# ketanfatania/QMRI-PnP-Recon-POC

Measured on AMD Instinct MI355X. Metric: ADMM iters/sec (224x224x10 TSMI, spiral mask), higher is better.
Workload: dtype f32; 1 GPU; cut3 224x224x10 single slice per GPU, spiral mask S=771 T=200, PnP-ADMM + 10-channel UNetRes (DRUNet) denoiser; solver=lsqr, admm_iters=20, dc_dtype=f64, parallelism=slice-parallel x1 (no collective)

## Files before the change

### qmri_pnp_recon_poc_amd/csrc/api_core.cpp

```cpp
#include "qmri_internal.h"
#include "fft_codelets.h"

#include <algorithm>
#include <atomic>
#include <cmath>
#include <cstdarg>
#include <cstdlib>
#include <cstring>
#include <mutex>

static thread_local std::string g_create_err;

namespace {
struct KnobDef { const char* name; int dflt; };
const KnobDef g_knob_defs[K_COUNT] = {
    {"conv_scheme", 2}, {"conv_f32", 0}, {"conv_wt", 1}, {"conv_xcd", 1}, {"conv_persist", 1}, {"conv_splitk", 1},
    {"conv_midcfg", 3}, {"conv_deepcfg", 3}, {"conv_deepks", 4},
    {"conv_resident", 1}, {"res_head", 1}, {"res_tail", 1}, {"res_down", 1}, {"res_delay", 24}, {"res_rearm", 64},
    {"res_stamps", 0}, {"conv_stamps", 0}, {"conv_stamp_launch", -1}, {"lsqr_stamps", 0},
    {"conv_mt2", 1024}, {"conv_occ", 2},
    {"fuse_ew", 1}, {"lsqr_persist", 1}, {"lsqr_fold", 1}, {"dictw_lsp", 2}, {"verbose", 0},
    {"pack_gpu", 1}, {"nufft_seg", NU_SEG},
    {"fmap_fuse", 0}, {"fmap_start", 0},
};
std::atomic<int> g_knob_val[K_COUNT];
std::once_flag g_knob_once;

int knob_index(const char* name, size_t len) {
    for (int k = 0; k < K_COUNT; ++k)
        if (strlen(g_knob_defs[k].name) == len && strncmp(g_knob_defs[k].name, name, len) == 0) return k;
    return -1;
}
void knob_init() {
    for (int k = 0; k < K_COUNT; ++k) g_knob_val[k].store(g_knob_defs[k].dflt, std::memory_order_relaxed);
    const char* e = getenv("QMRI_DEBUG");
    while (e && *e) {
        const char* end = strchr(e, ',');
        const size_t len = end ? (size_t)(end - e) : strlen(e);
        const char* eq = (const char*)memchr(e, '=', len);
        const int k = eq ? knob_index(e, (size_t)(eq - e)) : -1;
        if (k >= 0) g_knob_val[k].store(atoi(eq + 1), std::memory_order_relaxed);
// ... 822 lines not shown
```

### qmri_pnp_recon_poc_amd/csrc/api_net.cpp

```cpp
#include "qmri_internal.h"

#include <algorithm>
#include <chrono>
#include <cmath>
#include <cstdio>
#include <cstring>

extern "C" size_t qmri_net_nparams(const qmri_net_desc* d) {
    if (!d) return 0;
    size_t n = 0;
    if (d->arch == QMRI_ARCH_UNETRES) {
        const int32_t* nc = d->nc;
        n += (size_t)nc[0] * d->in_nc * 9;
        for (int l = 0; l < 3; ++l) n += (size_t)2 * d->nb * nc[l] * nc[l] * 9 + (size_t)nc[l + 1] * nc[l] * 4;
        n += (size_t)2 * d->nb * nc[3] * nc[3] * 9;
        for (int l = 3; l > 0; --l) n += (size_t)nc[l] * nc[l - 1] * 4 + (size_t)2 * d->nb * nc[l - 1] * nc[l - 1] * 9;
        n += (size_t)d->out_nc * nc[0] * 9;
    } else if (d->arch == QMRI_ARCH_SEQ_CONV) {
        if (d->nb == 1) return (size_t)d->out_nc * d->in_nc * 9;
        n = (size_t)d->nc[0] * d->in_nc * 9 + (size_t)(d->nb - 2) * d->nc[0] * d->nc[0] * 9 + (size_t)d->out_nc * d->nc[0] * 9;
    }
    return n;
}

// ... 250 lines not shown
        for (int l = 0; l < 3; ++l) {
            for (int b = 0; b < 2 * nb; ++b) QMRI_TRY(add_layer_timed(ctx, CONV_3X3, nc[l], nc[l], w));
            QMRI_TRY(add_layer_timed(ctx, CONV_DOWN, nc[l], nc[l + 1], w));
        }
        for (int b = 0; b < 2 * nb; ++b) QMRI_TRY(add_layer_timed(ctx, CONV_3X3, nc[3], nc[3], w));
        for (int l = 3; l > 0; --l) {
            QMRI_TRY(add_layer_timed(ctx, CONV_UP, nc[l], nc[l - 1], w));
            for (int b = 0; b < 2 * nb; ++b) QMRI_TRY(add_layer_timed(ctx, CONV_3X3, nc[l - 1], nc[l - 1], w));
        }
        QMRI_TRY(add_layer_timed(ctx, CONV_3X3, nc[0], desc->out_nc, w));
        for (int l = 0; l < 4; ++l) {
            int cal = conv_cin_pad(CONV_3X3, nc[l]);
            if (l < 3) cal = std::max(cal, conv_cin_pad(CONV_DOWN, nc[l]));
            if (l > 0) cal = std::max(cal, conv_cin_pad(CONV_UP, nc[l]));
            QMRI_TRY(alloc_tensor(ctx, p.x[l], nc[l], cal, H >> l, W >> l, B));
            QMRI_TRY(alloc_tensor(ctx, p.a[l], nc[l], cal, H >> l, W >> l, B));
            QMRI_TRY(alloc_tensor(ctx, p.t[l], nc[l], cal, H >> l, W >> l, B));
        }
        if (nc[0] == 64 && H % 16 == 0 && W % 16 == 0 && (H / 16) * (W / 16) <= 1024) {
            p.res_tiles = (H / 16) * (W / 16);
            QMRI_TRY(dev_alloc(ctx, &p.d_res_xbuf, conv6r_xbuf_bytes(p.res_tiles)));
            QMRI_HIP(ctx, hipMemset(p.d_res_xbuf, 0, conv6r_xbuf_bytes(p.res_tiles)));
            p.res_epoch = 0; p.res_off = false;
            if (qmri_knob(K_RES_STAMPS)) { QMRI_HIP(ctx, hipMalloc(&p.d_res_stamps, 1024 * sizeof(unsigned long long))); QMRI_HIP(ctx, hipMemset(p.d_res_stamps, 0, 1024 * sizeof(unsigned long long))); }
        }
    } else {
        const int width = desc->nc[0];
        if (nb == 1) QMRI_TRY(add_layer_timed(ctx, CONV_3X3, desc->in_nc, desc->out_nc, w));
        else {
            QMRI_TRY(add_layer_timed(ctx, CONV_3X3, desc->in_nc, width, w));
            for (int l = 1; l < nb - 1; ++l) QMRI_TRY(add_layer_timed(ctx, CONV_3X3, width, width, w));
            QMRI_TRY(add_layer_timed(ctx, CONV_3X3, width, desc->out_nc, w));
        }
        QMRI_TRY(alloc_tensor(ctx, p.a[0], width, conv_cin_pad(CONV_3X3, width), H, W, B));
        QMRI_TRY(alloc_tensor(ctx, p.t[0], width, conv_cin_pad(CONV_3X3, width), H, W, B));
    }
    if (p.d_wflat) {
        const auto t0 = Clk::now();
        QMRI_TRY(net_pack_all_dev(ctx));
        QMRI_HIP(ctx, hipStreamSynchronize(ctx->stream));
        ms_pack += std::chrono::duration<double, std::milli>(Clk::now() - t0).count();
    }
    p.w_begin = nullptr;
    QMRI_TRY(alloc_tensor(ctx, p.in32, desc->in_nc, conv_cin_pad(CONV_3X3, desc->in_nc), H, W, B));
    QMRI_TRY(alloc_tensor(ctx, p.out32, desc->out_nc, desc->out_nc, H, W, B));
    p.blk_ok = conv6_enabled();
    for (const ConvLayer& L : p.layers) if (!L.wp6) p.blk_ok = false;
// ... 231 lines not shown
    auto pass = [&]() -> int {
        if (hipMemcpyAsync(d_io, in, nin * sizeof(double), hipMemcpyHostToDevice, ctx->stream) != hipSuccess) return QMRI_ERR_HIP;
        QMRI_TRY(ew_launch_pack(ctx, B, C, H, W, d_io, 1, p.in32, in_scale));
        QMRI_TRY(net_forward(ctx, B));
        QMRI_TRY(ew_launch_unpack(ctx, B, p.desc.out_nc, H, W, p.out32, p.in32, p.desc.residual_noise, d_io, 1, out_scale));
        if (hipMemcpyAsync(out, d_io, nout * sizeof(double), hipMemcpyDeviceToHost, ctx->stream) != hipSuccess) return QMRI_ERR_HIP;
        if (hipStreamSynchronize(ctx->stream) != hipSuccess) return QMRI_ERR_HIP;
        return net_range_tripped(ctx, again);
    };
    int st = QMRI_OK;
    for (int attempt = 0; attempt < 3; ++attempt) {
        again = false;
        st = pass();
        if (st != QMRI_OK || !again) break;
    }
    if (st == QMRI_OK && again) { qmri_set_error(ctx, "the network's guards asked for a fourth pass (resident-tile hand-off / f16 range): giving up"); st = QMRI_ERR_HIP; }
    if (st == QMRI_ERR_HIP && ctx->err.empty()) qmri_set_error(ctx, "HIP failure in qmri_denoise");
    return st;
}

extern "C" int qmri_debug_conv_stamps(qmri_ctx* ctx, unsigned long long* out, int nwg) {
    if (ctx && nwg == -6 && ctx->net.d_res_stamps) {
        QMRI_HIP(ctx, hipStreamSynchronize(ctx->stream));
        QMRI_HIP(ctx, hipMemcpy(out, ctx->net.d_res_stamps, (size_t)1024 * sizeof(unsigned long long), hipMemcpyDeviceToHost));
        return QMRI_OK;
    }
    if (!ctx || !ctx->net.d_stamps) return QMRI_ERR_STATE;
    QMRI_HIP(ctx, hipStreamSynchronize(ctx->stream));
    QMRI_HIP(ctx, hipMemcpy(out, ctx->net.d_stamps, (size_t)4096 * 11 * sizeof(unsigned long long), hipMemcpyDeviceToHost));
    return QMRI_OK;
}
```

### qmri_pnp_recon_poc_amd/csrc/conv6r_kernels.hip

```cpp
#include "conv6_device.h"

namespace {

constexpr int R_MAXL = 10;
constexpr int R_RELU = 1;
constexpr int R_ADD = 2;
constexpr int R_SKIP = 4;
constexpr int R_STORE = 8;
constexpr int R_STORE_WT = 16;
constexpr int R_KEEP = 32;
constexpr int R_DOWN = 128;
constexpr unsigned R_DOWN_STEPB = 2 * 2 * 2 * 64 * 16;
constexpr int R_LOCAL = 256;
constexpr int R_TAIL = 64;
constexpr int R_IH = 18, R_IW = 18, R_IHP = 24;
constexpr int R_NPX = R_IHP * (R_IW - 1) + R_IH;
constexpr int R_CHUNK = 2 * 2 * R_NPX;
constexpr int R_AST = ast6(2);
constexpr int R_SPIN_MAX = 1 << 16;
constexpr int R_SEGT = 86, R_CORT = 6;
constexpr int R_NTRI = 4 * R_SEGT + 4 * R_CORT;
constexpr size_t conv6r_lds() { return (size_t)(NABUF * R_AST + 4 * R_CHUNK) * 16; }

struct Conv6rArgs {
    const float* src; const float* skip;
    const float* radd[R_MAXL]; float* sdst[R_MAXL];
    float* dn_out; int dn_hp, dn_plane;
    float* out; int out_hp, out_plane, out_c;
    int in_planar, in_plane;
    int nch[R_MAXL], kind[R_MAXL];
    unsigned char* xbuf; size_t xbuf_half;
    const uint4* wp[R_MAXL];
    float dh[R_MAXL], dl[R_MAXL];
    int am_layer[R_MAXL];
    int nlayers, hp, plane, tiles_h, tiles_w, xcd;
    int drop;
    int delay;
    unsigned epoch;
    unsigned* range_flag; float* am_slots; int* am_count;
    unsigned long long* stamps;
};

template <int N> __device__ __forceinline__ void gwait_a(u32x4 (&a)[3]) { asm volatile("s_waitcnt vmcnt(%3)" : "+v"(a[0]), "+v"(a[1]), "+v"(a[2]) : "n"(N) : "memory"); }
template <int IMM> __device__ __forceinline__ void gload4r_sc1(f32x4& dst, unsigned off, const void* base) { asm volatile("global_load_dwordx4 %0, %1, %2 offset:%3 sc1" : "=v"(dst) : "v"(off), "s"(base), "n"(IMM) : "memory"); }
template <int IMM> __device__ __forceinline__ void gstore4r(unsigned off, f32x4 x, void* base) { asm volatile("global_store_dwordx4 %0, %1, %2 offset:%3\n\ts_nop 1" ::"v"(off), "v"(x), "s"(base), "n"(IMM) : "memory"); }
template <int IMM> __device__ __forceinline__ void gstore4r_sc1(unsigned off, f32x4 x, void* base) { asm volatile("global_store_dwordx4 %0, %1, %2 offset:%3 sc1\n\ts_nop 1" ::"v"(off), "v"(x), "s"(base), "n"(IMM) : "memory"); }

__device__ __forceinline__ void r_tri_decode(int t, int& seg, int& j) {
    if (t < 4 * R_SEGT) { seg = t / R_SEGT; j = t - seg * R_SEGT; } else { seg = 4 + (t - 4 * R_SEGT) / R_CORT; j = (t - 4 * R_SEGT) - (seg - 4) * R_CORT; }
}
__device__ __forceinline__ int r_seg_base(int seg) { return seg < 4 ? seg * R_SEGT : 4 * R_SEGT + (seg - 4) * R_CORT; }
__device__ __forceinline__ unsigned r_ent_lds(int k, int dw, int dh) {
    const int cb = k >> 1, sp = k & 1;
    return (unsigned)(((cb >> 1) * R_CHUNK + sp * 2 * R_NPX + (cb & 1) * R_NPX + dw * R_IHP + dh) * 16);
}

#define R_STAMP(role, k)                                                                                         \
    do {                                                                                                         \
        if constexpr (STAMP) {                                                                                   \
            if (A.stamps && (threadIdx.x & 255) == 0 && blockIdx.x % 50 == 0 && blockIdx.x / 50 < 4)             \
                A.stamps[(((blockIdx.x / 50) * 2 + (role)) * R_MAXL + l) * 8 + (k)] = wall_clock64();            \
        }                                                                                                        \
    } while (0)
template <bool STAMP>
__global__ __launch_bounds__(NT6) void k_conv6r(const Conv6rArgs A) {
    constexpr int SP = 2, AST = R_AST, IHP = R_IHP, NPX = R_NPX, NAQ = 3;
    static_assert(AST == NAQ * NLD6, "one weight step = three 16-byte entries per loader thread");
    extern __shared__ __align__(16) unsigned char smem[];
    uint4* Abuf = (uint4*)smem;
    uint4* Bt = Abuf + NABUF * AST;
    const int tid = threadIdx.x;
    const int bid = A.xcd ? xcd_remap(blockIdx.x, gridDim.x) : blockIdx.x;
    const int th = bid % A.tiles_h, tw = bid / A.tiles_h;
    const int oh0 = th * 16, ow0 = tw * 16;
    const int nl = A.nlayers;
    const unsigned plane32 = (unsigned)A.plane * 32u;
    const unsigned tile0 = (unsigned)((ow0 * A.hp + oh0) * 32);

    if (tid >= NT6 - NLD6) {
        const int lt = tid - (NT6 - NLD6);
        __builtin_amdgcn_s_setprio(2);
        constexpr unsigned ASTB = AST * 16;
        unsigned aoff[NAQ];
#pragma unroll
        for (int q = 0; q < NAQ; ++q) aoff[q] = (unsigned)((lt + NLD6 * q) * 16);
        int rq_l = 0, rq_s = 0, rq_n = 3 * A.nch[0];
// ... 72 lines not shown
                                   "+v"(v[2][2]), "+v"(v[2][3]), "+v"(v[2][4]), "+v"(v[2][5]), "+v"(v[2][6]), "+v"(v[2][7])::"memory");
#pragma unroll
                    for (int k = 0; k < NQ; ++k) {
                        uint4 s0, s1;
                        split_pair_h(v[k][0], v[k][1], s0.x, s1.x);
                        split_pair_h(v[k][2], v[k][3], s0.y, s1.y);
                        split_pair_h(v[k][4], v[k][5], s0.z, s1.z);
                        split_pair_h(v[k][6], v[k][7], s0.w, s1.w);
                        if (lo[k] != ~0u) {
                            *(uint4*)((unsigned char*)Bt + lo[k]) = s0;
                            *(uint4*)((unsigned char*)Bt + lo[k] + 2 * NPX * 16) = s1;
                        }
                    }
                }
            }
            gwait_a<0>(ra0); gwait_a<0>(pa1);
            R_STORE_A(0, ra0) R_STORE_A(1, pa1)
        }
        unsigned p_lds[2][3], p_x[2];
#pragma unroll
        for (int q = 0; q < 2; ++q) {
            const int t = lt + NLD6 * q;
            const bool valid = t < R_NTRI;
            int seg, j;
            r_tri_decode(valid ? t : 0, seg, j);
            const int npx = seg < 4 ? 16 : 1;
#pragma unroll
            for (int i = 0; i < 3; ++i) {
                const int E = 3 * j + i, Ec = (E < npx * 16) ? E : 0, pp = Ec >> 4, k = Ec & 15;
                const int w = (seg == 0) ? 0 : (seg == 1) ? 15 : (seg == 2 || seg == 3) ? pp : (seg < 6 ? 0 : 15);
                const int h = (seg == 0 || seg == 1) ? pp : (seg == 2) ? 0 : (seg == 3) ? 15 : ((seg & 1) ? 15 : 0);
                p_lds[q][i] = r_ent_lds(k, w + 1, h + 1);
            }
            p_x[q] = valid ? (unsigned)((tw * A.tiles_h + th) * (R_NTRI * 64) + t * 16) : ~0u;
        }
        lds_barrier6();
#define R_ITER(k_, rs_, rq_)               \
        {                                                                                                        \
            __builtin_amdgcn_s_setprio(2);                                                                       \
            R_REQ(rq_)                                                                                           \
            __builtin_amdgcn_s_setprio(0);                                                                       \
            gwait_a<2 * NAQ>(rs_);                                                                               \
            R_STORE_A(((k_) + 2) % NABUF, rs_)                                                                   \
            lds_barrier6();                                                                                      \
        }
#pragma unroll 1
        for (int l = 0; l < nl; ++l) {
#pragma unroll 1
            for (int g = 0; g < 3 * A.nch[l]; g += 3) {
                R_ITER(0, ra1, ra0)
                R_ITER(1, ra2, ra1)
                R_ITER(2, ra0, ra2)
            }
            R_STAMP(1, 0);
            if (A.kind[l] & R_TAIL) {
                lds_barrier6();
                const float* tl = (const float*)Bt;
                const unsigned opx = (unsigned)(((ow0 + (lt >> 4) + 1) * A.out_hp + (oh0 + (lt & 15)) + 1) * 4), opl = (unsigned)A.out_plane * 4u;
                for (int c = 0; c < A.out_c; ++c) {
                    const float x = tl[c * 256 + lt];
                    asm volatile("global_store_dword %0, %1, %2" ::"v"(opx + (unsigned)c * opl), "v"(x), "s"(A.out) : "memory");
                }
                break;
            }
            if (!(A.kind[l] & R_KEEP)) break;
            lds_barrier6();
            if (A.kind[l] & R_LOCAL) continue;
            R_STAMP(1, 1);
            const unsigned tag = (A.epoch + (unsigned)l + 1u) & 0xFFFFu, thi = tag << 16;
            unsigned char* xb = A.xbuf + (size_t)(l & 1) * A.xbuf_half;
            if (!(A.drop && th == 0 && tw == 0)) {
#pragma unroll
                for (int q = 0; q < 2; ++q) {
                    if (p_x[q] == ~0u) continue;
                    unsigned d[12];
#pragma unroll
                    for (int i = 0; i < 3; ++i) {
                        const uint4 e = *(const uint4*)((const unsigned char*)Bt + p_lds[q][i]);
                        d[4 * i] = e.x; d[4 * i + 1] = e.y; d[4 * i + 2] = e.z; d[4 * i + 3] = e.w;
                    }
#pragma unroll
                    for (int i = 0; i < 4; ++i) {
                        u32x4 g;
                        g[0] = d[3 * i];
                        g[1] = (d[3 * i + 1] & 0xFFFFu) | thi;
                        g[2] = (d[3 * i + 1] >> 16) | (d[3 * i + 2] << 16);
                        g[3] = (d[3 * i + 2] >> 16) | thi;
                        asm volatile("global_store_dwordx4 %0, %1, %2 sc1\n\ts_nop 1" ::"v"(p_x[q] + (unsigned)(i * (R_NTRI * 16))), "v"(g), "s"(xb) : "memory");
                    }
                }
            }
            R_STAMP(1, 2);
            R_STAMP(1, 5);
            lds_barrier6();
            R_STAMP(1, 6);
        }
        gwait_a<0>(ra0); gwait_a<0>(ra1); gwait_a<0>(ra2);
#undef R_ITER
#undef R_REQ
#undef R_STORE_A
        return;
    }
    const int wave = tid >> 6, lane = tid & 63, li = lane & 31, h2 = lane >> 5;
    const int pbw = 4 * wave;
    const int pxl = (pbw + (li >> 3)) * IHP + (li & 7);
    const unsigned gpx = (unsigned)(((ow0 + pbw + (li >> 3) + 1) * A.hp + (oh0 + (li & 7)) + 1) * 32 + 16 * h2);
    bool dead = false;
    lds_barrier6();
#pragma unroll 1
    for (int l = 0; l < nl; ++l) {
        R_STAMP(0, 0);
        f32x16 acc[2][2], accl[2][2];
#pragma unroll
        for (int m = 0; m < 2; ++m)
#pragma unroll
            for (int n = 0; n < 2; ++n)
#pragma unroll
// ... 144 lines not shown
                    go += plane32;                                                                               \
                }                                                                                                \
        }
#define R_ADD_OPERAND()                            \
        {                                                                                                        \
            asm volatile("s_waitcnt vmcnt(0)"                                                                    \
                         : "+v"(res[0][0][0]), "+v"(res[0][0][1]), "+v"(res[0][0][2]), "+v"(res[0][0][3]), "+v"(res[0][1][0]), "+v"(res[0][1][1]), \
                           "+v"(res[0][1][2]), "+v"(res[0][1][3]), "+v"(res[1][0][0]), "+v"(res[1][0][1]), "+v"(res[1][0][2]), "+v"(res[1][0][3]), \
                           "+v"(res[1][1][0]), "+v"(res[1][1][1]), "+v"(res[1][1][2]), "+v"(res[1][1][3])::"memory");     \
            _Pragma("unroll") for (int m = 0; m < 2; ++m)                                                        \
                _Pragma("unroll") for (int n = 0; n < 2; ++n)                                                    \
                    _Pragma("unroll") for (int r = 0; r < 16; r += 2) {                                          \
                        const f32x2 x = pair(m, n, r) + f32x2{res[m][n][r >> 2][r & 3], res[m][n][r >> 2][(r & 3) + 1]}; \
                        acc[m][n][r] = x[0]; acc[m][n][r + 1] = x[1];                                            \
                    }                                                                                            \
        }
        if (kind & R_ADD) { R_REQ_OPERAND(A.radd[l]) R_ADD_OPERAND() }
        if (kind & R_SKIP) { R_REQ_OPERAND(A.skip) R_ADD_OPERAND() }
#undef R_REQ_OPERAND
#undef R_ADD_OPERAND
        R_STAMP(0, 2);
        float gmax = 0.f;
        bool bad = false;
        auto finish = [&](auto relu_c, auto store_c, auto keep_c) __attribute__((always_inline)) {
            constexpr bool RELU = decltype(relu_c)::value, KEEP = decltype(keep_c)::value;
            constexpr int STORE = decltype(store_c)::value;
            float* sd = A.sdst[l];
            unsigned go = gpx_l;
#pragma unroll
            for (int m = 0; m < 2; ++m)
#pragma unroll
                for (int rg = 0; rg < 4; ++rg) {
#pragma unroll
                    for (int n = 0; n < 2; ++n) {
                        f32x4 x;
#pragma unroll
                        for (int j = 0; j < 4; ++j) { x[j] = acc[m][n][4 * rg + j]; if constexpr (RELU) x[j] = fmaxf(x[j], 0.f); }
                        const float gm = fmaxf(fmaxf(fabsf(x[0]), fabsf(x[1])), fmaxf(fabsf(x[2]), fabsf(x[3])));
                        bad |= !(gm <= F16_RANGE);
                        gmax = fmaxf(gmax, gm);
                        if constexpr (KEEP) {
                            uint2 s0, s1;
                            split_pair_h(x[0], x[1], s0.x, s1.x);
                            split_pair_h(x[2], x[3], s0.y, s1.y);
                            unsigned char* bd = (unsigned char*)Bt + (((2 * m + (rg >> 1)) * R_CHUNK + (rg & 1) * NPX + pxl_l + IHP + 1 + 8 * n) * 16 + 8 * h2_l);
                            *(uint2*)bd = s0;
                            *(uint2*)(bd + 2 * NPX * 16) = s1;
                        }
                        if constexpr (STORE != 0) {
                            if constexpr (STORE == 2) { if (n) gstore4r_sc1<256>(go, x, sd); else gstore4r_sc1<0>(go, x, sd); } else { if (n) gstore4r<256>(go, x, sd); else gstore4r<0>(go, x, sd); }
                        }
                    }
                    go += plane32;
                }
        };
        typedef std::true_type T1; typedef std::false_type T0;
        typedef std::integral_constant<int, 0> S0; typedef std::integral_constant<int, 1> S1; typedef std::integral_constant<int, 2> S2;
        if ((kind & R_RELU) && (kind & R_KEEP)) finish(T1{}, S0{}, T1{});
        else if ((kind & R_STORE) && (kind & R_KEEP)) finish(T0{}, S1{}, T1{});
        else if (kind & R_STORE_WT) finish(T0{}, S2{}, T0{});
        else finish(T0{}, S0{}, T1{});
        if (bad && A.range_flag) atomicOr(A.range_flag, 1u);
        act_report(ActMax{A.am_slots, A.am_count, A.am_layer[l]}, gmax, 4);
        R_STAMP(0, 3);
        if (!(kind & R_KEEP)) break;
        lds_barrier6();
        if (kind & R_LOCAL) continue;
        R_STAMP(0, 4);
        {
            int tid_l = tid;
            asm volatile("" : "+v"(tid_l));
            unsigned c_lds[2][3], c_x[2];
#pragma unroll
            for (int q = 0; q < 2; ++q) {
                const int t = tid_l + 256 * q;
                const bool valid = t < R_NTRI;
                int seg, j;
                r_tri_decode(valid ? t : 0, seg, j);
                const int npx = seg < 4 ? 16 : 1;
                const int dtw = (seg == 0 || seg == 4 || seg == 5) ? -1 : (seg == 1 || seg == 6 || seg == 7) ? 1 : 0;
                const int dth = (seg == 2 || seg == 4 || seg == 6) ? -1 : (seg == 3 || seg == 5 || seg == 7) ? 1 : 0;
                const int ns = (seg < 4) ? (seg ^ 1) : 11 - seg;
                const bool have = valid && tw + dtw >= 0 && tw + dtw < A.tiles_w && th + dth >= 0 && th + dth < A.tiles_h;
#pragma unroll
                for (int i = 0; i < 3; ++i) {
                    const int E = 3 * j + i, pp = E >> 4, k = E & 15;
                    const int dw = (dtw < 0) ? 0 : (dtw > 0) ? 17 : pp + 1, dh = (dth < 0) ? 0 : (dth > 0) ? 17 : pp + 1;
                    c_lds[q][i] = (have && E < npx * 16) ? r_ent_lds(k, dw, dh) : ~0u;
                }
                c_x[q] = have ? (unsigned)(((tw + dtw) * A.tiles_h + th + dth) * (R_NTRI * 64) + (r_seg_base(ns) + j) * 16) : ~0u;
            }
            const unsigned tag = (A.epoch + (unsigned)l + 1u) & 0xFFFFu, thi = tag << 16;
            const unsigned char* xb = A.xbuf + (size_t)(l & 1) * A.xbuf_half;
            for (int i = 0; i < A.delay; ++i) __builtin_amdgcn_s_sleep(1);
            {
                bool pend[2] = {c_x[0] != ~0u && !dead, c_x[1] != ~0u && !dead};
                bool ok = false;
                for (int spin = 0; spin < R_SPIN_MAX; ++spin) {
                    u32x4 g[2][4];
#pragma unroll
                    for (int q = 0; q < 2; ++q)
                        if (pend[q]) {
#pragma unroll
                            for (int i = 0; i < 4; ++i) asm volatile("global_load_dwordx4 %0, %1, %2 sc1" : "=v"(g[q][i]) : "v"(c_x[q] + (unsigned)(i * (R_NTRI * 16))), "s"(xb) : "memory");
                        }
                    asm volatile("s_waitcnt vmcnt(0)" : "+v"(g[0][0]), "+v"(g[0][1]), "+v"(g[0][2]), "+v"(g[0][3]), "+v"(g[1][0]), "+v"(g[1][1]), "+v"(g[1][2]), "+v"(g[1][3])::"memory");
#pragma unroll
                    for (int q = 0; q < 2; ++q)
                        if (pend[q]) {
                            unsigned bad = 0;
#pragma unroll
                            for (int i = 0; i < 4; ++i) bad |= (g[q][i][1] ^ thi) | (g[q][i][3] ^ thi);
                            if ((bad >> 16) == 0) {
                                unsigned d[12];
#pragma unroll
                                for (int i = 0; i < 4; ++i) {
                                    d[3 * i] = g[q][i][0];
                                    d[3 * i + 1] = (g[q][i][1] & 0xFFFFu) | (g[q][i][2] << 16);
                                    d[3 * i + 2] = (g[q][i][2] >> 16) | (g[q][i][3] << 16);
                                }
#pragma unroll
                                for (int i = 0; i < 3; ++i)
                                    if (c_lds[q][i] != ~0u) *(uint4*)((unsigned char*)Bt + c_lds[q][i]) = make_uint4(d[4 * i], d[4 * i + 1], d[4 * i + 2], d[4 * i + 3]);
                                pend[q] = false;
                            }
                        }
                    if (!__any(pend[0] || pend[1])) { ok = true; break; }
                    __builtin_amdgcn_s_sleep(1);
                }
                if (!ok && !dead) { dead = true; if (lane == 0 && A.range_flag) atomicOr(A.range_flag, 4u); }
            }
        }
        R_STAMP(0, 5);
        lds_barrier6();
        R_STAMP(0, 6);
    }
}

}

int conv6r_try(qmri_ctx* ctx, const Conv6rRun& run, int B, bool* done) {
    *done = false;
    NetPlan& net = ctx->net;
    hipStreamCaptureStatus cap = hipStreamCaptureStatusNone;
    const bool capturing = hipStreamIsCapturing(ctx->stream, &cap) == hipSuccess && cap != hipStreamCaptureStatusNone;
    const int nres = run.nres, nl = nres + (run.head ? 1 : 0) + (run.tail ? 1 : 0) + (run.down ? 1 : 0);
    if (!qmri_knob(K_CONV_RESIDENT) || capturing || net.res_off || !net.d_res_xbuf || B != 1 || nres < 2 || nl > R_MAXL || (nres & 1) || net.d_stamps) return QMRI_OK;
    if (!run.res || !run.src || !run.cur || (run.head && (!run.head_in || run.skip)) || (run.tail && !run.tail_out) || (run.down && (!run.down_out || run.tail || run.skip))) return QMRI_OK;
    auto is3 = [](const ConvLayer& L) { return (L.kind == CONV_3X3 || L.kind == CONV_3X3N) && L.sp6 == 2 && L.wp6 && L.n_ct6 == 1; };
    for (int l = 0; l < nres; ++l) {
        const ConvLayer& L = run.res[l];
        if (!is3(L) || L.Cin != 64 || L.Cout != 64 || L.nchunk6 != 4) return QMRI_OK;
    }
    const PTensor &src = *run.src, &cur = *run.cur;
    const PTensor* ts[3] = {&src, &cur, run.skip};
    for (const PTensor* t : ts) {
        if (!t) continue;
// ... 35 lines not shown
    int l = 0;
    auto put = [&](const ConvLayer& L, int kind, const float* radd, float* sdst) {
        A.wp[l] = reinterpret_cast<const uint4*>(L.wp6);
        A.dh[l] = L.w6_descale; A.dl[l] = L.w6_descale * (1.f / LO_SCALE);
        A.am_layer[l] = conv6_act_slot(ctx, true, L).layer;
        A.nch[l] = L.nchunk6; A.kind[l] = kind; A.radd[l] = radd; A.sdst[l] = sdst;
        ++l;
    };
    if (run.head) put(*run.head, R_STORE | R_KEEP, nullptr, src.fbase());
    for (int r = 0; r < nres; ++r) {
        const bool last = r == nres - 1;
        if (!(r & 1)) put(run.res[r], R_RELU | R_KEEP, nullptr, nullptr);
        else if (!last) put(run.res[r], R_ADD | R_STORE | R_KEEP, (r == 1) ? src.fbase() : cur.fbase(), cur.fbase());
        else if (run.tail) put(run.res[r], R_ADD | (run.skip ? R_SKIP : 0) | R_KEEP, (r == 1) ? src.fbase() : cur.fbase(), nullptr);
        else if (run.down) put(run.res[r], R_ADD | R_KEEP | R_LOCAL, (r == 1) ? src.fbase() : cur.fbase(), nullptr);
        else put(run.res[r], R_ADD | (run.skip ? R_SKIP : 0) | R_STORE_WT, (r == 1) ? src.fbase() : cur.fbase(), cur.fbase());
    }
    if (run.tail) put(*run.tail, R_TAIL, nullptr, nullptr);
    if (run.down) { put(*run.down, R_DOWN, nullptr, nullptr); A.nch[l - 1] = 6; }
    for (int k = l; k < R_MAXL; ++k) { A.wp[k] = A.wp[l - 1]; A.nch[k] = A.nch[l - 1]; A.am_layer[k] = -1; }
    int pub[2] = {0, 0};
    for (int k = 0; k < l; ++k) if ((A.kind[k] & R_KEEP) && !(A.kind[k] & R_LOCAL)) pub[k & 1] += 1;
    if (!pub[0] || !pub[1]) return QMRI_OK;
    A.nlayers = nl; A.hp = src.hp; A.plane = (int)src.plane(); A.tiles_h = tiles_h; A.tiles_w = tiles_w;
    A.xbuf = net.d_res_xbuf; A.xbuf_half = (size_t)tiles * R_NTRI * 64;
    A.xcd = qmri_knob(K_CONV_XCD);
    const int delay = std::max(0, std::min(4096, qmri_knob(K_RES_DELAY)));
    A.epoch = net.res_epoch; A.drop = net.res_drop; A.delay = delay;
    A.range_flag = net.d_range_flag; A.am_slots = net.d_act_slots; A.am_count = net.d_act_count;
    if (!ctx->conv6r_attr) {
        QMRI_HIP(ctx, hipFuncSetAttribute((const void*)k_conv6r<false>, hipFuncAttributeMaxDynamicSharedMemorySize, (int)conv6r_lds()));
        QMRI_HIP(ctx, hipFuncSetAttribute((const void*)k_conv6r<true>, hipFuncAttributeMaxDynamicSharedMemorySize, (int)conv6r_lds()));
        ctx->conv6r_attr = true;
    }
    g_conv6_launch_counter.fetch_add(nl, std::memory_order_relaxed);
    const int stamp_which = qmri_knob(K_RES_STAMPS);
    A.stamps = (stamp_which == 2) == (run.head != nullptr) ? (unsigned long long*)net.d_res_stamps : nullptr;
    hipEvent_t e0 = nullptr, e1 = nullptr;
    double flop = 0.0;
    for (int r = 0; r < nres; ++r) flop += conv_layer_flop(run.res[r], 1, src.H, src.W);
    if (run.head) flop += conv_layer_flop(*run.head, 1, src.H, src.W);
    if (run.tail) flop += conv_layer_flop(*run.tail, 1, src.H, src.W);
    if (run.down) flop += conv_layer_flop(*run.down, 1, src.H, src.W);
    QMRI_TRY(qmri_prof_pair(ctx, &e0, &e1, PROF_CONV3, flop));
    if (A.stamps) k_conv6r<true><<<dim3(tiles), dim3(NT6), conv6r_lds(), ctx->stream>>>(A);
    else if (e0) hipExtLaunchKernelGGL((k_conv6r<false>), dim3(tiles), dim3(NT6), (std::uint32_t)conv6r_lds(), ctx->stream, e0, e1, 0, A);
    else k_conv6r<false><<<dim3(tiles), dim3(NT6), conv6r_lds(), ctx->stream>>>(A);
    QMRI_HIP(ctx, hipGetLastError());
    net.res_epoch += (unsigned)(nl - 1);
    *done = true;
    return QMRI_OK;
// ... 4 lines not shown
```

### qmri_pnp_recon_poc_amd/csrc/qmri_internal.h

```cpp
#pragma once

#include <hip/hip_runtime.h>
#include <algorithm>
#include <cstdint>
#include <cstdio>
#include <string>
#include <vector>

#include "../../include/qmri.h"

struct qmri_ctx;
void qmri_set_error(qmri_ctx* ctx, const char* fmt, ...);

#define QMRI_HIP(ctx, expr)                                                                       \
    do {                                                                                          \
        hipError_t _e = (expr);                                                                   \
        if (_e != hipSuccess) {                                                                   \
            qmri_set_error((ctx), "%s failed: %s (%s:%d)", #expr, hipGetErrorString(_e), __FILE__, __LINE__); \
            return QMRI_ERR_HIP;                                                                  \
        }                                                                                         \
    } while (0)

#define QMRI_CHECK_ARG(ctx, cond, msg)                                                            \
    do {                                                                                          \
// ... 33 lines not shown
    Stream() = default; Stream(Stream&& o) noexcept : s(o.s) { o.s = nullptr; }
    ~Stream() { if (s) (void)hipStreamDestroy(s); }
    operator hipStream_t() const { return s; }
};
template <typename T> int dev_alloc(qmri_ctx* ctx, T** p, size_t count) {
    *p = nullptr;
    hipError_t e = hipMalloc((void**)p, std::max<size_t>(count, 1) * sizeof(T));
    if (e != hipSuccess) { qmri_set_error(ctx, "hipMalloc of %zu bytes failed: %s", count * sizeof(T), hipGetErrorString(e)); return QMRI_ERR_NOMEM; }
    return QMRI_OK;
}
}

enum QmriKnob {
    K_CONV_SCHEME,
    K_CONV_F32,
    K_CONV_WT,
    K_CONV_XCD,
    K_CONV_PERSIST,
    K_CONV_SPLITK,
    K_CONV_MIDCFG, K_CONV_DEEPCFG, K_CONV_DEEPKS,
    K_CONV_RESIDENT,
    K_RES_HEAD, K_RES_TAIL, K_RES_DOWN,
    K_RES_DELAY,
    K_RES_REARM,
    K_RES_STAMPS, K_CONV_STAMPS, K_CONV_STAMP_LAUNCH, K_LSQR_STAMPS,
    K_CONV_MT2, K_CONV_OCC,
    K_FUSE_EW,
    K_LSQR_PERSIST,
    K_LSQR_FOLD,
    K_DICTW_LSP,
    K_VERBOSE,
    K_PACK_GPU,
    K_NUFFT_SEG,
    K_FMAP_FUSE,
    K_FMAP_START,
    K_COUNT
};
int qmri_knob(QmriKnob k);

struct KEntry {
    uint16_t kw;
    uint16_t t;
};


struct OpDev {
// ... 495 lines not shown
```

Baseline: 814.8 ADMM iters/s.

## Pipeline resident-conv halo exchange chunk-by-chunk with next layer's channel loop

Reorganizes the halo ring buffer in the resident conv kernel so boundary data is grouped by channel chunk. With the new res_pipe knob on by default, chunk 0 of the halo is published and fetched at the layer boundary, and chunks 1-3 are fetched inside the next layer's channel loop, overlapped with A-operand loads. It also drops the trailing barrier after publication. The goal is to hide inter-tile halo exchange latency and remove a barrier, at the cost of extra spin-wait logic, more polling traffic, and a restriction to layers with exactly four channel chunks.

```diff
diff --git a/qmri_pnp_recon_poc_amd/csrc/api_core.cpp b/qmri_pnp_recon_poc_amd/csrc/api_core.cpp
--- a/qmri_pnp_recon_poc_amd/csrc/api_core.cpp
+++ b/qmri_pnp_recon_poc_amd/csrc/api_core.cpp
@@ -16,7 +16,7 @@
 const KnobDef g_knob_defs[K_COUNT] = {
     {"conv_scheme", 2}, {"conv_f32", 0}, {"conv_wt", 1}, {"conv_xcd", 1}, {"conv_persist", 1}, {"conv_splitk", 1},
     {"conv_midcfg", 3}, {"conv_deepcfg", 3}, {"conv_deepks", 4},
-    {"conv_resident", 1}, {"res_head", 1}, {"res_tail", 1}, {"res_down", 1}, {"res_delay", 24}, {"res_rearm", 64},
+    {"conv_resident", 1}, {"res_head", 1}, {"res_tail", 1}, {"res_down", 1}, {"res_delay", 24}, {"res_pipe", 1}, {"res_pipe_delay", 8}, {"res_rearm", 64},
     {"res_stamps", 0}, {"conv_stamps", 0}, {"conv_stamp_launch", -1}, {"lsqr_stamps", 0},
     {"conv_mt2", 1024}, {"conv_occ", 2},
     {"fuse_ew", 1}, {"lsqr_persist", 1}, {"lsqr_fold", 1}, {"dictw_lsp", 2}, {"verbose", 0},
diff --git a/qmri_pnp_recon_poc_amd/csrc/api_net.cpp b/qmri_pnp_recon_poc_amd/csrc/api_net.cpp
--- a/qmri_pnp_recon_poc_amd/csrc/api_net.cpp
+++ b/qmri_pnp_recon_poc_amd/csrc/api_net.cpp
@@ -296,7 +296,7 @@
             QMRI_TRY(dev_alloc(ctx, &p.d_res_xbuf, conv6r_xbuf_bytes(p.res_tiles)));
             QMRI_HIP(ctx, hipMemset(p.d_res_xbuf, 0, conv6r_xbuf_bytes(p.res_tiles)));
             p.res_epoch = 0; p.res_off = false;
-            if (qmri_knob(K_RES_STAMPS)) { QMRI_HIP(ctx, hipMalloc(&p.d_res_stamps, 1024 * sizeof(unsigned long long))); QMRI_HIP(ctx, hipMemset(p.d_res_stamps, 0, 1024 * sizeof(unsigned long long))); }
+            if (qmri_knob(K_RES_STAMPS)) { QMRI_HIP(ctx, hipMalloc(&p.d_res_stamps, 2048 * sizeof(unsigned long long))); QMRI_HIP(ctx, hipMemset(p.d_res_stamps, 0, 2048 * sizeof(unsigned long long))); }
         }
     } else {
         const int width = desc->nc[0];
@@ -574,7 +574,7 @@
 extern "C" int qmri_debug_conv_stamps(qmri_ctx* ctx, unsigned long long* out, int nwg) {
     if (ctx && nwg == -6 && ctx->net.d_res_stamps) {
         QMRI_HIP(ctx, hipStreamSynchronize(ctx->stream));
-        QMRI_HIP(ctx, hipMemcpy(out, ctx->net.d_res_stamps, (size_t)1024 * sizeof(unsigned long long), hipMemcpyDeviceToHost));
+        QMRI_HIP(ctx, hipMemcpy(out, ctx->net.d_res_stamps, (size_t)2048 * sizeof(unsigned long long), hipMemcpyDeviceToHost));
         return QMRI_OK;
     }
     if (!ctx || !ctx->net.d_stamps) return QMRI_ERR_STATE;
diff --git a/qmri_pnp_recon_poc_amd/csrc/conv6r_kernels.hip b/qmri_pnp_recon_poc_amd/csrc/conv6r_kernels.hip
--- a/qmri_pnp_recon_poc_amd/csrc/conv6r_kernels.hip
+++ b/qmri_pnp_recon_poc_amd/csrc/conv6r_kernels.hip
@@ -1,4 +1,5 @@
 #include "conv6_device.h"
+#include "conv6r_ring.h"
 
 namespace {
 
@@ -13,13 +14,9 @@
 constexpr unsigned R_DOWN_STEPB = 2 * 2 * 2 * 64 * 16;
 constexpr int R_LOCAL = 256;
 constexpr int R_TAIL = 64;
-constexpr int R_IH = 18, R_IW = 18, R_IHP = 24;
-constexpr int R_NPX = R_IHP * (R_IW - 1) + R_IH;
-constexpr int R_CHUNK = 2 * 2 * R_NPX;
 constexpr int R_AST = ast6(2);
 constexpr int R_SPIN_MAX = 1 << 16;
-constexpr int R_SEGT = 86, R_CORT = 6;
-constexpr int R_NTRI = 4 * R_SEGT + 4 * R_CORT;
+static_assert(R_NTRI <= 2 * NLD6 && R_CHT <= NLD6, "two triples per thread to publish, one per thread and chunk to fetch");
 constexpr size_t conv6r_lds() { return (size_t)(NABUF * R_AST + 4 * R_CHUNK) * 16; }
 
 struct Conv6rArgs {
@@ -35,7 +32,9 @@
     int am_layer[R_MAXL];
     int nlayers, hp, plane, tiles_h, tiles_w, xcd;
     int drop;
+    int pipe;
     int delay;
+    int pdelay;
     unsigned epoch;
     unsigned* range_flag; float* am_slots; int* am_count;
     unsigned long long* stamps;
@@ -46,22 +45,14 @@
 template <int IMM> __device__ __forceinline__ void gstore4r(unsigned off, f32x4 x, void* base) { asm volatile("global_store_dwordx4 %0, %1, %2 offset:%3\n\ts_nop 1" ::"v"(off), "v"(x), "s"(base), "n"(IMM) : "memory"); }
 template <int IMM> __device__ __forceinline__ void gstore4r_sc1(unsigned off, f32x4 x, void* base) { asm volatile("global_store_dwordx4 %0, %1, %2 offset:%3 sc1\n\ts_nop 1" ::"v"(off), "v"(x), "s"(base), "n"(IMM) : "memory"); }
 
-__device__ __forceinline__ void r_tri_decode(int t, int& seg, int& j) {
-    if (t < 4 * R_SEGT) { seg = t / R_SEGT; j = t - seg * R_SEGT; } else { seg = 4 + (t - 4 * R_SEGT) / R_CORT; j = (t - 4 * R_SEGT) - (seg - 4) * R_CORT; }
-}
-__device__ __forceinline__ int r_seg_base(int seg) { return seg < 4 ? seg * R_SEGT : 4 * R_SEGT + (seg - 4) * R_CORT; }
-__device__ __forceinline__ unsigned r_ent_lds(int k, int dw, int dh) {
-    const int cb = k >> 1, sp = k & 1;
-    return (unsigned)(((cb >> 1) * R_CHUNK + sp * 2 * R_NPX + (cb & 1) * R_NPX + dw * R_IHP + dh) * 16);
-}
-
-#define R_STAMP(role, k)                                                                                         \
+#define R_STAMPV(role, k, v)                                                                                     \
     do {                                                                                                         \
         if constexpr (STAMP) {                                                                                   \
             if (A.stamps && (threadIdx.x & 255) == 0 && blockIdx.x % 50 == 0 && blockIdx.x / 50 < 4)             \
-                A.stamps[(((blockIdx.x / 50) * 2 + (role)) * R_MAXL + l) * 8 + (k)] = wall_clock64();            \
+                A.stamps[(((blockIdx.x / 50) * 2 + (role)) * R_MAXL + l) * 16 + (k)] = (v);                      \
         }                                                                                                        \
     } while (0)
+#define R_STAMP(role, k) R_STAMPV(role, k, wall_clock64())
 template <bool STAMP>
 __global__ __launch_bounds__(NT6) void k_conv6r(const Conv6rArgs A) {
     constexpr int SP = 2, AST = R_AST, IHP = R_IHP, NPX = R_NPX, NAQ = 3;
@@ -180,18 +171,81 @@
         for (int q = 0; q < 2; ++q) {
             const int t = lt + NLD6 * q;
             const bool valid = t < R_NTRI;
-            int seg, j;
-            r_tri_decode(valid ? t : 0, seg, j);
-            const int npx = seg < 4 ? 16 : 1;
+            const int tc = valid ? t : 0, ck = r_tri_chunk(tc), seg = r_tri_seg(tc), j = r_tri_j(tc);
+#pragma unroll
+            for (int i = 0; i < 3; ++i) p_lds[q][i] = r_pub_lds_d(ck, seg, j, i);
+            p_x[q] = valid ? r_slot(t, th, tw, A.tiles_h) : R_NONE;
+        }
+        unsigned f_lds[3], f_x;
+        {
+            const bool fv = lt < R_CHT;
+            const int seg = r_tri_seg(fv ? lt : 0), j = r_tri_j(fv ? lt : 0);
+            const bool have = (int(fv) & int(r_ring_have_d(seg, th, tw, A.tiles_h, A.tiles_w))) != 0;
+#pragma unroll
+            for (int i = 0; i < 3; ++i) f_lds[i] = r_ring_lds_d(0, seg, j, i, have);
+            const unsigned fs = r_ring_slot_d(0, seg, j, th, tw, A.tiles_h, have);
+            f_x = fs != R_NONE ? fs : r_slot(0, th, tw, A.tiles_h);
+        }
+        const unsigned f_idle = r_slot(0, th, tw, A.tiles_h);
+        bool dead = false;
+        auto publish = [&](auto qc, unsigned thi, unsigned char* xb) __attribute__((always_inline)) {
+            constexpr int q = decltype(qc)::value;
+            unsigned d[12];
 #pragma unroll
             for (int i = 0; i < 3; ++i) {
-                const int E = 3 * j + i, Ec = (E < npx * 16) ? E : 0, pp = Ec >> 4, k = Ec & 15;
-                const int w = (seg == 0) ? 0 : (seg == 1) ? 15 : (seg == 2 || seg == 3) ? pp : (seg < 6 ? 0 : 15);
-                const int h = (seg == 0 || seg == 1) ? pp : (seg == 2) ? 0 : (seg == 3) ? 15 : ((seg & 1) ? 15 : 0);
-                p_lds[q][i] = r_ent_lds(k, w + 1, h + 1);
-            }
-            p_x[q] = valid ? (unsigned)((tw * A.tiles_h + th) * (R_NTRI * 64) + t * 16) : ~0u;
-        }
+                const uint4 e = *(const uint4*)((const unsigned char*)Bt + p_lds[q][i]);
+                d[4 * i] = e.x; d[4 * i + 1] = e.y; d[4 * i + 2] = e.z; d[4 * i + 3] = e.w;
+            }
+#pragma unroll
+            for (int i = 0; i < 4; ++i) {
+                u32x4 g;
+                g[0] = d[3 * i];
+                g[1] = (d[3 * i + 1] & 0xFFFFu) | thi;
+                g[2] = (d[3 * i + 1] >> 16) | (d[3 * i + 2] << 16);
+                g[3] = (d[3 * i + 2] >> 16) | thi;
+                const unsigned po = p_x[q] + (unsigned)(i * (R_NTRI * 16));
+                asm volatile("global_store_dwordx4 %0, %1, %2 sc1\n\ts_nop 1" ::"v"(po), "v"(g), "s"(xb) : "memory");
+            }
+        };
+        auto ring_req = [&](u32x4 (&g)[4], unsigned slot, const unsigned char* xb) __attribute__((always_inline)) {
+#pragma unroll
+            for (int i = 0; i < 4; ++i) {
+                const unsigned fo = slot + (unsigned)(i * (R_NTRI * 16));
+                asm volatile("global_load_dwordx4 %0, %1, %2 sc1" : "=v"(g[i]) : "v"(fo), "s"(xb) : "memory");
+            }
+        };
+        auto ring_take = [&](const u32x4 (&g)[4], int c, unsigned thi) __attribute__((always_inline)) -> bool {
+            unsigned bad = 0;
+#pragma unroll
+            for (int i = 0; i < 4; ++i) bad |= (g[i][1] ^ thi) | (g[i][3] ^ thi);
+            if ((bad >> 16) != 0) return false;
+            unsigned d[12];
+#pragma unroll
+            for (int i = 0; i < 4; ++i) {
+                d[3 * i] = g[i][0];
+                d[3 * i + 1] = (g[i][1] & 0xFFFFu) | (g[i][2] << 16);
+                d[3 * i + 2] = (g[i][2] >> 16) | (g[i][3] << 16);
+            }
+#pragma unroll
+            for (int i = 0; i < 3; ++i)
+                if (f_lds[i] != R_NONE) *(uint4*)((unsigned char*)Bt + f_lds[i] + (unsigned)(c * (R_CHUNK * 16))) = make_uint4(d[4 * i], d[4 * i + 1], d[4 * i + 2], d[4 * i + 3]);
+            return true;
+        };
+        auto ring_spin = [&](bool pend, int c, unsigned thi, const unsigned char* xb) __attribute__((always_inline)) -> int {
+            int spin = 0;
+            bool ok = false;
+            for (; spin < R_SPIN_MAX; ++spin) {
+                u32x4 g[4];
+                if (pend) ring_req(g, f_x + (unsigned)(c * (R_CHT * 16)), xb);
+                asm volatile("s_waitcnt vmcnt(0)" : "+v"(g[0]), "+v"(g[1]), "+v"(g[2]), "+v"(g[3])::"memory");
+                if (pend && ring_take(g, c, thi)) pend = false;
+                if (!__any(pend)) { ok = true; break; }
+                __builtin_amdgcn_s_sleep(1);
+            }
+            if (!ok) { dead = true; if ((lt & 63) == 0 && A.range_flag) atomicOr(A.range_flag, 4u); }
+            return spin;
+        };
+        typedef std::integral_constant<int, 0> Q0; typedef std::integral_constant<int, 1> Q1;
         lds_barrier6();
 #define R_ITER(k_, rs_, rq_)               \
         {                                                                                                        \
@@ -204,13 +258,43 @@
         }
 #pragma unroll 1
         for (int l = 0; l < nl; ++l) {
+            const bool fin = A.pipe && l > 0 && (A.kind[l - 1] & (R_KEEP | R_LOCAL)) == R_KEEP;
+            const unsigned thip = ((A.epoch + (unsigned)l) & 0xFFFFu) << 16;
+            const unsigned char* xbp = A.xbuf + (size_t)((l + 1) & 1) * A.xbuf_half;
+            int nretry = 0;
 #pragma unroll 1
             for (int g = 0; g < 3 * A.nch[l]; g += 3) {
+                const int c = g / 3 + 1;
+                const bool fnow = fin && c < 4;
+                u32x4 rg[4];
                 R_ITER(0, ra1, ra0)
-                R_ITER(1, ra2, ra1)
-                R_ITER(2, ra0, ra2)
+                {
+                    __builtin_amdgcn_s_setprio(2);
+                    ring_req(rg, fnow ? f_x + (unsigned)(c * (R_CHT * 16)) : f_idle, xbp);
+                    R_REQ(ra1)
+                    __builtin_amdgcn_s_setprio(0);
+                    gwait_a<2 * NAQ + 4>(ra2);
+                    R_STORE_A(0, ra2)
+                    lds_barrier6();
+                }
+                {
+                    __builtin_amdgcn_s_setprio(2);
+                    R_REQ(ra2)
+                    __builtin_amdgcn_s_setprio(0);
+                    asm volatile("s_waitcnt vmcnt(%7)" : "+v"(ra0[0]), "+v"(ra0[1]), "+v"(ra0[2]), "+v"(rg[0]), "+v"(rg[1]), "+v"(rg[2]), "+v"(rg[3]) : "n"(2 * NAQ) : "memory");
+                    if (fnow) {
+                        bool pend = f_lds[0] != R_NONE && !dead;
+                        if (pend && ring_take(rg, c, thip)) pend = false;
+                        if (__any(pend)) nretry += 1 + ring_spin(pend, c, thip, xbp);
+                        R_STAMP(1, 7 + c);
+                    }
+                    R_STORE_A(1, ra0)
+                    lds_barrier6();
+                    if (fnow) R_STAMP(1, 10 + c);
+                }
             }
             R_STAMP(1, 0);
+            R_STAMPV(1, 15, (unsigned long long)nretry);
             if (A.kind[l] & R_TAIL) {
                 lds_barrier6();
                 const float* tl = (const float*)Bt;
@@ -222,35 +306,34 @@
                 break;
             }
             if (!(A.kind[l] & R_KEEP)) break;
-            lds_barrier6();
-            if (A.kind[l] & R_LOCAL) continue;
-            R_STAMP(1, 1);
+            const bool pubs = !(A.kind[l] & R_LOCAL);
+            const bool silent = A.drop && th == 0 && tw == 0;
             const unsigned tag = (A.epoch + (unsigned)l + 1u) & 0xFFFFu, thi = tag << 16;
             unsigned char* xb = A.xbuf + (size_t)(l & 1) * A.xbuf_half;
-            if (!(A.drop && th == 0 && tw == 0)) {
-#pragma unroll
-                for (int q = 0; q < 2; ++q) {
-                    if (p_x[q] == ~0u) continue;
-                    unsigned d[12];
-#pragma unroll
-                    for (int i = 0; i < 3; ++i) {
-                        const uint4 e = *(const uint4*)((const unsigned char*)Bt + p_lds[q][i]);
-                        d[4 * i] = e.x; d[4 * i + 1] = e.y; d[4 * i + 2] = e.z; d[4 * i + 3] = e.w;
-                    }
-#pragma unroll
-                    for (int i = 0; i < 4; ++i) {
-                        u32x4 g;
-                        g[0] = d[3 * i];
-                        g[1] = (d[3 * i + 1] & 0xFFFFu) | thi;
-                        g[2] = (d[3 * i + 1] >> 16) | (d[3 * i + 2] << 16);
-                        g[3] = (d[3 * i + 2] >> 16) | thi;
-                        asm volatile("global_store_dwordx4 %0, %1, %2 sc1\n\ts_nop 1" ::"v"(p_x[q] + (unsigned)(i * (R_NTRI * 16))), "v"(g), "s"(xb) : "memory");
-                    }
-                }
+            if (A.pipe && pubs) {
+                lds_barrier6();
+                R_STAMP(1, 3);
+                if (!silent && lt < R_CHT) publish(Q0{}, thi, xb);
+                R_STAMP(1, 4);
+                const bool pend = f_lds[0] != R_NONE && !dead;
+                int ns = 0;
+                if (__any(pend)) {
+                    for (int i = 0; i < A.pdelay; ++i) __builtin_amdgcn_s_sleep(1);
+                    ns = ring_spin(pend, 0, thi, xb);
+                }
+                R_STAMP(1, 7);
+                R_STAMPV(1, 14, (unsigned long long)ns);
+            }
+            lds_barrier6();
+            if (!pubs) continue;
+            R_STAMP(1, 1);
+            if (!silent) {
+                if (!(A.pipe && lt < R_CHT)) publish(Q0{}, thi, xb);
+                if (p_x[1] != R_NONE) publish(Q1{}, thi, xb);
             }
             R_STAMP(1, 2);
             R_STAMP(1, 5);
-            lds_barrier6();
+            if (!A.pipe) lds_barrier6();
             R_STAMP(1, 6);
         }
         gwait_a<0>(ra0); gwait_a<0>(ra1); gwait_a<0>(ra2);
@@ -441,6 +524,7 @@
         R_STAMP(0, 2);
         float gmax = 0.f;
         bool bad = false;
+        const bool e1a = A.pipe && (kind & (R_KEEP | R_LOCAL)) == R_KEEP;
         auto finish = [&](auto relu_c, auto store_c, auto keep_c) __attribute__((always_inline)) {
             constexpr bool RELU = decltype(relu_c)::value, KEEP = decltype(keep_c)::value;
             constexpr int STORE = decltype(store_c)::value;
@@ -471,6 +555,12 @@
                         }
                     }
                     go += plane32;
+                    if constexpr (KEEP) {
+                        if (m == 0 && rg == 1 && e1a) {
+                            lds_barrier6();
+                            R_STAMP(0, 7);
+                        }
+                    }
                 }
         };
         typedef std::true_type T1; typedef std::false_type T0;
@@ -486,7 +576,7 @@
         lds_barrier6();
         if (kind & R_LOCAL) continue;
         R_STAMP(0, 4);
-        {
+        if (!A.pipe) {
             int tid_l = tid;
             asm volatile("" : "+v"(tid_l));
             unsigned c_lds[2][3], c_x[2];
@@ -494,20 +584,11 @@
             for (int q = 0; q < 2; ++q) {
                 const int t = tid_l + 256 * q;
                 const bool valid = t < R_NTRI;
-                int seg, j;
-                r_tri_decode(valid ? t : 0, seg, j);
-                const int npx = seg < 4 ? 16 : 1;
-                const int dtw = (seg == 0 || seg == 4 || seg == 5) ? -1 : (seg == 1 || seg == 6 || seg == 7) ? 1 : 0;
-                const int dth = (seg == 2 || seg == 4 || seg == 6) ? -1 : (seg == 3 || seg == 5 || seg == 7) ? 1 : 0;
-                const int ns = (seg < 4) ? (seg ^ 1) : 11 - seg;
-                const bool have = valid && tw + dtw >= 0 && tw + dtw < A.tiles_w && th + dth >= 0 && th + dth < A.tiles_h;
-#pragma unroll
-                for (int i = 0; i < 3; ++i) {
-                    const int E = 3 * j + i, pp = E >> 4, k = E & 15;
-                    const int dw = (dtw < 0) ? 0 : (dtw > 0) ? 17 : pp + 1, dh = (dth < 0) ? 0 : (dth > 0) ? 17 : pp + 1;
-                    c_lds[q][i] = (have && E < npx * 16) ? r_ent_lds(k, dw, dh) : ~0u;
-                }
-                c_x[q] = have ? (unsigned)(((tw + dtw) * A.tiles_h + th + dth) * (R_NTRI * 64) + (r_seg_base(ns) + j) * 16) : ~0u;
+                const int tc = valid ? t : 0, ck = r_tri_chunk(tc), seg = r_tri_seg(tc), j = r_tri_j(tc);
+                const bool have = (int(valid) & int(r_ring_have_d(seg, th, tw, A.tiles_h, A.tiles_w))) != 0;
+#pragma unroll
+                for (int i = 0; i < 3; ++i) c_lds[q][i] = r_ring_lds_d(ck, seg, j, i, have);
+                c_x[q] = r_ring_slot_d(ck, seg, j, th, tw, A.tiles_h, have);
             }
             const unsigned tag = (A.epoch + (unsigned)l + 1u) & 0xFFFFu, thi = tag << 16;
             const unsigned char* xb = A.xbuf + (size_t)(l & 1) * A.xbuf_half;
@@ -551,7 +632,7 @@
             }
         }
         R_STAMP(0, 5);
-        lds_barrier6();
+        if (!A.pipe) lds_barrier6();
         R_STAMP(0, 6);
     }
 }
@@ -633,11 +714,14 @@
     int pub[2] = {0, 0};
     for (int k = 0; k < l; ++k) if ((A.kind[k] & R_KEEP) && !(A.kind[k] & R_LOCAL)) pub[k & 1] += 1;
     if (!pub[0] || !pub[1]) return QMRI_OK;
+    for (int k = 1; k < l; ++k)
+        if ((A.kind[k - 1] & (R_KEEP | R_LOCAL)) == R_KEEP && A.nch[k] != 4) return QMRI_OK;
     A.nlayers = nl; A.hp = src.hp; A.plane = (int)src.plane(); A.tiles_h = tiles_h; A.tiles_w = tiles_w;
     A.xbuf = net.d_res_xbuf; A.xbuf_half = (size_t)tiles * R_NTRI * 64;
     A.xcd = qmri_knob(K_CONV_XCD);
     const int delay = std::max(0, std::min(4096, qmri_knob(K_RES_DELAY)));
     A.epoch = net.res_epoch; A.drop = net.res_drop; A.delay = delay;
+    A.pipe = qmri_knob(K_RES_PIPE) ? 1 : 0; A.pdelay = std::max(0, std::min(4096, qmri_knob(K_RES_PIPE_DELAY)));
     A.range_flag = net.d_range_flag; A.am_slots = net.d_act_slots; A.am_count = net.d_act_count;
     if (!ctx->conv6r_attr) {
         QMRI_HIP(ctx, hipFuncSetAttribute((const void*)k_conv6r<false>, hipFuncAttributeMaxDynamicSharedMemorySize, (int)conv6r_lds()));
diff --git a/qmri_pnp_recon_poc_amd/csrc/conv6r_ring.h b/qmri_pnp_recon_poc_amd/csrc/conv6r_ring.h
--- /dev/null
+++ b/qmri_pnp_recon_poc_amd/csrc/conv6r_ring.h
@@ -0,0 +1,58 @@
+#pragma once
+#if defined(__HIPCC__)
+#define R_HD __host__ __device__ constexpr
+#else
+#define R_HD constexpr
+#endif
+
+constexpr int R_IH = 18, R_IW = 18, R_IHP = 24;
+constexpr int R_NPX = R_IHP * (R_IW - 1) + R_IH;
+constexpr int R_CHUNK = 2 * 2 * R_NPX;
+constexpr int R_SEGT = 22, R_CORT = 2;
+constexpr int R_CHT = 4 * R_SEGT + 4 * R_CORT;
+constexpr int R_NTRI = 4 * R_CHT;
+
+R_HD int r_tri_chunk(int t) { return t / R_CHT; }
+R_HD int r_tri_seg(int t) { return int((t % R_CHT) < 4 * R_SEGT) * ((t % R_CHT) / R_SEGT) + int((t % R_CHT) >= 4 * R_SEGT) * (4 + ((t % R_CHT) - 4 * R_SEGT) / R_CORT); }
+R_HD int r_seg_base(int seg) { return int(seg < 4) * seg * R_SEGT + int(seg >= 4) * (4 * R_SEGT + (seg - 4) * R_CORT); }
+R_HD int r_tri_j(int t) { return (t % R_CHT) - r_seg_base(r_tri_seg(t)); }
+R_HD int r_tri_index(int chunk, int seg, int j) { return chunk * R_CHT + r_seg_base(seg) + j; }
+R_HD int r_seg_npx(int seg) { return 1 + 15 * int(seg < 4); }
+R_HD bool r_ent_valid(int seg, int j, int i) { return 3 * j + i < 4 * r_seg_npx(seg); }
+R_HD int r_ent_px(int j, int i) { return (3 * j + i) >> 2; }
+R_HD int r_ent_k(int chunk, int j, int i) { return 4 * chunk + ((3 * j + i) & 3); }
+R_HD unsigned r_ent_lds(int k, int dw, int dh) {
+    return (unsigned)((((k >> 1) >> 1) * R_CHUNK + (k & 1) * 2 * R_NPX + ((k >> 1) & 1) * R_NPX + dw * R_IHP + dh) * 16);
+}
+R_HD int r_pub_w(int seg, int pp) { return int(seg == 1) * 15 + int((seg | 1) == 3) * pp + int(seg >= 6) * 15; }
+R_HD int r_pub_h(int seg, int pp) { return int(seg < 2) * pp + int(seg == 3) * 15 + int(seg >= 4) * 15 * (seg & 1); }
+R_HD int r_nb_dtw(int seg) { return (int(seg == 1) | int(seg == 6) | int(seg == 7)) - (int(seg == 0) | int(seg == 4) | int(seg == 5)); }
+R_HD int r_nb_dth(int seg) { return (int(seg == 3) | int(seg == 5) | int(seg == 7)) - (int(seg == 2) | int(seg == 4) | int(seg == 6)); }
+R_HD int r_nb_seg(int seg) { return int(seg < 4) * (seg ^ 1) + int(seg >= 4) * (11 - seg); }
+R_HD int r_ring_dw(int seg, int pp) { return int(r_nb_dtw(seg) > 0) * 17 + int(r_nb_dtw(seg) == 0) * (pp + 1); }
+R_HD int r_ring_dh(int seg, int pp) { return int(r_nb_dth(seg) > 0) * 17 + int(r_nb_dth(seg) == 0) * (pp + 1); }
+
+constexpr unsigned R_NONE = ~0u;
+R_HD unsigned r_pub_lds_d(int chunk, int seg, int j, int i) {
+    return r_ent_valid(seg, j, i) ? r_ent_lds(r_ent_k(chunk, j, i), r_pub_w(seg, r_ent_px(j, i)) + 1, r_pub_h(seg, r_ent_px(j, i)) + 1) : r_ent_lds(4 * chunk, 1, 1);
+}
+R_HD unsigned r_pub_lds(int t, int i) { return r_pub_lds_d(r_tri_chunk(t), r_tri_seg(t), r_tri_j(t), i); }
+R_HD bool r_ring_have_d(int seg, int th, int tw, int tiles_h, int tiles_w) {
+    return (int(tw + r_nb_dtw(seg) >= 0) & int(tw + r_nb_dtw(seg) < tiles_w) & int(th + r_nb_dth(seg) >= 0) & int(th + r_nb_dth(seg) < tiles_h)) != 0;
+}
+R_HD bool r_ring_have(int t, int th, int tw, int tiles_h, int tiles_w) { return r_ring_have_d(r_tri_seg(t), th, tw, tiles_h, tiles_w); }
+R_HD unsigned r_ring_lds_d(int chunk, int seg, int j, int i, bool have) {
+    return (int(have) & int(r_ent_valid(seg, j, i))) ? r_ent_lds(r_ent_k(chunk, j, i), r_ring_dw(seg, r_ent_px(j, i)), r_ring_dh(seg, r_ent_px(j, i))) : R_NONE;
+}
+R_HD unsigned r_ring_lds(int t, int i, int th, int tw, int tiles_h, int tiles_w) {
+    return r_ring_lds_d(r_tri_chunk(t), r_tri_seg(t), r_tri_j(t), i, r_ring_have(t, th, tw, tiles_h, tiles_w));
+}
+R_HD unsigned r_slot(int t, int th, int tw, int tiles_h) { return (unsigned)((tw * tiles_h + th) * (R_NTRI * 64) + t * 16); }
+R_HD unsigned r_ring_slot_d(int chunk, int seg, int j, int th, int tw, int tiles_h, bool have) {
+    return have ? r_slot(r_tri_index(chunk, r_nb_seg(seg), j), th + r_nb_dth(seg), tw + r_nb_dtw(seg), tiles_h) : R_NONE;
+}
+R_HD unsigned r_ring_slot(int t, int th, int tw, int tiles_h, int tiles_w) {
+    return r_ring_slot_d(r_tri_chunk(t), r_tri_seg(t), r_tri_j(t), th, tw, tiles_h, r_ring_have(t, th, tw, tiles_h, tiles_w));
+}
+R_HD int r_pub_thread(int t) { return t & 255; }
+R_HD int r_pub_turn(int t) { return t >> 8; }
diff --git a/qmri_pnp_recon_poc_amd/csrc/qmri_internal.h b/qmri_pnp_recon_poc_amd/csrc/qmri_internal.h
--- a/qmri_pnp_recon_poc_amd/csrc/qmri_internal.h
+++ b/qmri_pnp_recon_poc_amd/csrc/qmri_internal.h
@@ -79,6 +79,8 @@
     K_CONV_RESIDENT,
     K_RES_HEAD, K_RES_TAIL, K_RES_DOWN,
     K_RES_DELAY,
+    K_RES_PIPE,
+    K_RES_PIPE_DELAY,
     K_RES_REARM,
     K_RES_STAMPS, K_CONV_STAMPS, K_CONV_STAMP_LAUNCH, K_LSQR_STAMPS,
     K_CONV_MT2, K_CONV_OCC,
```

New measurement: 840.3 ADMM iters/s (median of 6 runs). +3.1%, better.
